# zcash/halo2

Hardware: AMD Instinct MI355X
Metric: Pallas MSM Mscalar-mults/s (+ Fp NTT Gbutterflies/s) at k=20 (higher is better)
Workload: dtype u256 (8x32-bit Montgomery limbs)

## Files before the change

halo2_amd/csrc/msm_fold.hip:

```cpp
#include "msm_internal.cuh"

namespace h2 {

template <int FB>
__global__ void __launch_bounds__(256) msm_finish_buckets(const u32 *__restrict__ heads, const u32 *__restrict__ starts,
                                                          u32 *__restrict__ buckets, u32 *__restrict__ heavy,
                                                          u32 total_buckets, u32 T, u32 div) {
    H2_LATENCY_STAGE();
    const u32 b = (blockIdx.x * blockDim.x + threadIdx.x) / kGroup;
    if (b >= total_buckets) return;
    const bool lead = (threadIdx.x & (kGroup - 1)) == 0;
    const u32 M = starts[total_buckets];
    T = eff_lanes(M, T, div);
    const u32 chunk = max(1u, (M + T - 1) / T);
    const u32 h0 = (starts[b] + chunk - 1) / chunk, h1 = (starts[b + 1] + chunk - 1) / chunk;
    if (h1 <= h0) return;
    if (h1 - h0 > kHeavy) {
        u32 slot = 0;
        if (lead) slot = atomicAdd(&heavy[1], 1u);
        slot = (u32)__builtin_amdgcn_mov_dpp((int)slot, 0, 0xf, 0xf, false);
        if (slot < kMaxHeavy) {
            if (lead) {
                heavy[2 + slot] = b;
                atomicAdd(&heavy[0], 1u);
// ... 99 lines not shown
        starts = H2_COLZ(starts, cs.starts);
        buckets9 = H2_COLZ(buckets9, cs.buckets);
        heavy = H2_COLZ(heavy, cs.heavy);
    }
    const u32 base = starts[0];
    const u32 M = starts[total_buckets] - base;
    T = eff_lanes(M, T, div);
    const u32 chunk = max(1u, (M + T - 1) / T);
    const u32 h0 = (starts[b] - base + chunk - 1) / chunk, h1 = (starts[b + 1] - base + chunk - 1) / chunk;
    if (h1 <= h0) return;
    if (h1 - h0 > kHeavy) {
        const u32 slot = atomicAdd(&heavy[1], 1u);
        if (slot < kMaxHeavy) {
            heavy[2 + slot] = b;
            atomicAdd(&heavy[0], 1u);
            return;
        }
    }
    xyzz9<FB> acc = xyzz9_load_raw<FB>(buckets9 + 36 * (size_t)b);
    for (u32 t = h0; t < h1; ++t) xyzz9_add<FB>(acc, xyzz9_load_raw<FB>(heads9 + 36 * (size_t)t));
    xyzz9_store_raw<FB>(buckets9 + 36 * (size_t)b, acc);
}
template <int FB>
__global__ void __launch_bounds__(256, 3) fold9_finish_heavy(const u32 *__restrict__ heads9, const u32 *__restrict__ starts, u32 *__restrict__ scratch9,
                                                          const u32 *__restrict__ heavy, u32 total_buckets, u32 T, u32 div, ColStride cs) {
    if (!cs.lowprio) H2_LATENCY_STAGE();
    __shared__ __attribute__((aligned(16))) u32 sh[32 * 36];
    if (gridDim.z > 1) {
        heavy = H2_COLZ(heavy, cs.heavy);
        heads9 = H2_COLZ(heads9, cs.heads);
        starts = H2_COLZ(starts, cs.starts);
        scratch9 = H2_COLZ(scratch9, cs.hscratch);
    }
    const u32 count = min(heavy[1], kMaxHeavy);
    const u32 base = starts[0];
    const u32 M = starts[total_buckets] - base;
    T = eff_lanes(M, T, div);
    const u32 chunk = max(1u, (M + T - 1) / T);
    for (u32 slot = blockIdx.y; slot < count; slot += gridDim.y) {
        const u32 b = heavy[2 + slot];
        const u32 h0 = (starts[b] - base + chunk - 1) / chunk, h1 = (starts[b + 1] - base + chunk - 1) / chunk;
        const u32 share = (h1 - h0 + kHeavyBlocks - 1) / kHeavyBlocks;
        const u32 lo = h0 + blockIdx.x * share, hi = min(h1, lo + share);
        xyzz9<FB> acc = fold9_quad_gather<FB, H2_FOLD_D>(heads9, hi > lo ? hi - lo : 0u, [lo](u32 k) { return lo + k; });
        acc = fold9_quads_sum<FB>(acc, sh);
        if (fold9_root() && (threadIdx.x & (kGroup - 1)) == 0) xyzz9_store_raw<FB>(scratch9 + 36 * ((size_t)slot * kHeavyBlocks + blockIdx.x), acc);
// ... 21 lines not shown
            if ((threadIdx.x & (kGroup - 1)) == 0) xyzz9_store_raw<FB>(buckets9 + 36 * (size_t)b, acc);
        }
        __syncthreads();
    }
}
template <int FB>
__global__ void __launch_bounds__(256, 3) fold9_rowcol(const u32 *__restrict__ buckets9, u32 *__restrict__ lines9, u32 S, u32 NR, ColStride cs) {
    if (!cs.lowprio) H2_LATENCY_STAGE();
    __shared__ __attribute__((aligned(16))) u32 sh[32 * 36];
    if (gridDim.z > 1) {
        buckets9 = H2_COLZ(buckets9, cs.buckets);
        lines9 = H2_COLZ(lines9, cs.lines);
    }
    const bool is_col = blockIdx.x < S;
    const u32 id = is_col ? blockIdx.x : blockIdx.x - S + 1;
    const u32 cnt = is_col ? NR : S;
    const u32 base = blockIdx.y * S * NR + (is_col ? id : id * S), step = is_col ? S : 1;
    xyzz9<FB> acc = fold9_quad_gather<FB, H2_FOLD_D>(buckets9, cnt, [base, step](u32 k) { return base + k * step; });
    acc = fold9_quads_sum<FB>(acc, sh);
    if (fold9_root() && (threadIdx.x & (kGroup - 1)) == 0)
        xyzz9_store_raw<FB>(lines9 + 36 * ((size_t)blockIdx.y * (S + NR) + (is_col ? id : S + id)), acc);
}
template <int FB>
__global__ void __launch_bounds__(256, 3) fold9_planes(const u32 *__restrict__ lines9, u32 *__restrict__ planes9, u32 *__restrict__ counter, u32 S, u32 NR,
                                                    int cb, u32 *__restrict__ out, int out_kind, int out_mont, ColOut co, ColStride cs) {
    if (!cs.lowprio) H2_LATENCY_STAGE();
    __shared__ __attribute__((aligned(16))) u32 sh[32 * 36];
    __shared__ u32 s_last;
    if (gridDim.z > 1) {
        lines9 = H2_COLZ(lines9, cs.lines);
        planes9 = H2_COLZ(planes9, cs.planes);
        counter = H2_COLZ(counter, cs.ctr);
        out = co.out[blockIdx.z];
    }
    const u32 t = blockIdx.x, planes = gridDim.x;
    const bool lead = (threadIdx.x & (kGroup - 1)) == 0;
    lines9 += 36 * (size_t)blockIdx.y * (S + NR);
    planes9 += 36 * (size_t)blockIdx.y * 32;
    counter += blockIdx.y;
    out += (out_kind == kOutSliceSum ? 32 : out_kind == H2_OUT_AFFINE ? 16 : 24) * (size_t)blockIdx.y;
    const u32 ncol = (int)t < cb ? S / 2 : (int)t == cb ? 1u : 0u, nrow = (int)t >= cb ? NR / 2 : 0u;
    const u32 jc = t, jr = t - (u32)cb;
    xyzz9<FB> acc = fold9_quad_gather<FB, H2_FOLD_D>(lines9, ncol + nrow, [=](u32 k) {
        if (k < ncol) {
            if ((int)jc == cb) return S - 1;
            return ((((k >> jc) << (jc + 1)) | (1u << jc) | (k & ((1u << jc) - 1u))) - 1u);
        }
        const u32 r = k - ncol;
        return S + (((r >> jr) << (jr + 1)) | (1u << jr) | (r & ((1u << jr) - 1u)));
    });
    acc = fold9_quads_sum<FB>(acc, sh);
    if (fold9_root()) {
        for (u32 k = 0; k < t; ++k) acc = xyzz9_dbl_wide<FB>(acc);
        if (lead) {
            xyzz9_store_raw<FB>(planes9 + 36 * (size_t)t, acc);
            __threadfence();
            s_last = atomicAdd(counter, 1u) == planes - 1 ? 1u : 0u;
        }
    }
    __syncthreads();
    if (!s_last) return;
    __threadfence();
    acc = fold9_quad_gather<FB, H2_FOLD_D>(planes9, planes, [](u32 k) { return k; });
    acc = fold9_quads_sum<FB>(acc, sh);
    if (!fold9_root()) return;
    const xyzz<FB> r = xyzz9_to_r256_wide<FB>(acc);
    if (!lead) return;
    *counter = 0;
    if (out_kind == kOutSliceSum) {
        xyzz_store<FB>(out, r);
        return;
    }
    if (out_kind == H2_OUT_AFFINE) {
        affine<FB> o = xyzz_to_affine<FB>(r);
        if (!out_mont) { o.x = fe_from_mont<FB>(o.x); o.y = fe_from_mont<FB>(o.y); }
        fe_store(out, o.x);
        fe_store(out + 8, o.y);
    } else {
        fe X, Y, Z;
        xyzz_to_jacobian<FB>(r, X, Y, Z);
        if (!out_mont) { X = fe_from_mont<FB>(X); Y = fe_from_mont<FB>(Y); Z = fe_from_mont<FB>(Z); }
        fe_store(out, X);
        fe_store(out + 8, Y);
        fe_store(out + 16, Z);
    }
}


template <int FB>
__global__ void __launch_bounds__(256) msm_reduce_segments(const u32 *__restrict__ buckets, u32 *__restrict__ partial,
// ... 57 lines not shown
    const size_t base = is_col ? id : (size_t)id * S, step = is_col ? S : 1;
    xyzz<FB> acc = xyzz_identity<FB>();
    for (u32 i = t; i < cnt; i += nl) {
        xyzz<FB> p = xyzz_load<FB>(buckets + 32 * (base + (size_t)i * step));
        xyzz_add_wide<FB>(acc, p);
    }
    if (lead) xyzz_store<FB>(sh + 32 * t, acc);
    __syncthreads();
    for (u32 off = nl / 2; off > 0; off >>= 1) {
        if (t < off) {
            xyzz<FB> a = xyzz_load<FB>(sh + 32 * t), b = xyzz_load<FB>(sh + 32 * (t + off));
            xyzz_add_wide<FB>(a, b);
            if (lead) xyzz_store<FB>(sh + 32 * t, a);
        }
        __syncthreads();
    }
    if (threadIdx.x == 0) {
        xyzz<FB> r = xyzz_load<FB>(sh);
        xyzz_store<FB>(wide + 32 * (is_col ? (size_t)id : (size_t)NR + id - 1), r);
    }
}

template <int FB>
__global__ void __launch_bounds__(64) msm_combine(const u32 *__restrict__ slice_sums, int slices, int c, u32 *__restrict__ out,
                                                  int out_kind, int out_mont, int extra_dbl, const u32 *__restrict__ addend, int addend_first) {
    H2_LATENCY_STAGE();
    if (threadIdx.x >= kGroup) return;
    if (gridDim.x > 1) {
        slice_sums += 32 * (size_t)blockIdx.x;
        out += (out_kind == H2_OUT_AFFINE ? 16 : 24) * (size_t)blockIdx.x;
        slices = 1;
    }
    xyzz9<FB> r9 = xyzz9_identity<FB>();
    for (int w = slices - 1; w >= 0; --w) {
        if (w != slices - 1)
            for (int k = 0; k < c; ++k) r9 = xyzz9_dbl_wide<FB>(r9);
        const xyzz9<FB> s9 = xyzz9_from_r256_wide<FB>(xyzz_load<FB>(slice_sums + 32 * (size_t)w));
        xyzz9_add_wide<FB>(r9, s9);
    }
    if (addend && addend_first) xyzz9_add_wide<FB>(r9, xyzz9_from_r256_wide<FB>(xyzz_load<FB>(addend)));
    for (int k = 0; k < extra_dbl; ++k) r9 = xyzz9_dbl_wide<FB>(r9);
    if (addend && !addend_first) xyzz9_add_wide<FB>(r9, xyzz9_from_r256_wide<FB>(xyzz_load<FB>(addend)));
    const xyzz<FB> r = xyzz9_to_r256_wide<FB>(r9);
    if (threadIdx.x != 0) return;
    if (out_kind == kOutSliceSum) {
        xyzz_store<FB>(out, r);
        return;
    }
    if (out_kind == H2_OUT_AFFINE) {
        affine<FB> a = xyzz_to_affine<FB>(r);
        if (!out_mont) { a.x = fe_from_mont<FB>(a.x); a.y = fe_from_mont<FB>(a.y); }
        fe_store(out, a.x);
        fe_store(out + 8, a.y);
    } else {
        fe X, Y, Z;
        xyzz_to_jacobian<FB>(r, X, Y, Z);
        if (!out_mont) { X = fe_from_mont<FB>(X); Y = fe_from_mont<FB>(Y); Z = fe_from_mont<FB>(Z); }
        fe_store(out, X);
        fe_store(out + 8, Y);
        fe_store(out + 16, Z);
    }
}

template <int FB>
__global__ void __launch_bounds__(64) msm_combine_ranges(RangeSums rs, int ranges, int slices, int c, u32 *__restrict__ out, int out_kind, int out_mont) {
    H2_LATENCY_STAGE();
    __shared__ __attribute__((aligned(16))) u32 sh[16 * 36];
    const int w = threadIdx.x / kGroup;
    const bool lead = (threadIdx.x & (kGroup - 1)) == 0;
    if (w < slices) {
        xyzz9<FB> acc = xyzz9_identity<FB>();
        for (int q = 0; q < ranges; ++q) xyzz9_add_wide<FB>(acc, xyzz9_from_r256_wide<FB>(xyzz_load<FB>(rs.p[q] + 32 * (size_t)w)));
        if (lead) xyzz9_store_raw<FB>(sh + 36 * w, acc);
    }
    __syncthreads();
    if (threadIdx.x >= kGroup) return;
    xyzz9<FB> r9 = xyzz9_identity<FB>();
    for (int s = slices - 1; s >= 0; --s) {
        if (s != slices - 1)
            for (int k = 0; k < c; ++k) r9 = xyzz9_dbl_wide<FB>(r9);
        xyzz9_add_wide<FB>(r9, xyzz9_load_raw<FB>(sh + 36 * s));
    }
    const xyzz<FB> r = xyzz9_to_r256_wide<FB>(r9);
    if (threadIdx.x != 0) return;
// ... 15 lines not shown

template __global__ void msm_finish_buckets<FP>(const u32 *__restrict__ heads, const u32 *__restrict__ starts,
                                                          u32 *__restrict__ buckets, u32 *__restrict__ heavy,
                                                          u32 total_buckets, u32 T, u32 div);
template __global__ void msm_finish_buckets<FQ>(const u32 *__restrict__ heads, const u32 *__restrict__ starts,
                                                          u32 *__restrict__ buckets, u32 *__restrict__ heavy,
                                                          u32 total_buckets, u32 T, u32 div);
template __global__ void msm_finish_heavy<FP>(const u32 *__restrict__ heads, const u32 *__restrict__ starts,
                                                        u32 *__restrict__ scratch, const u32 *__restrict__ heavy,
                                                        u32 total_buckets, u32 T, u32 div);
template __global__ void msm_finish_heavy<FQ>(const u32 *__restrict__ heads, const u32 *__restrict__ starts,
                                                        u32 *__restrict__ scratch, const u32 *__restrict__ heavy,
                                                        u32 total_buckets, u32 T, u32 div);
template __global__ void msm_finish_heavy2<FP>(const u32 *__restrict__ scratch, u32 *__restrict__ buckets,
                                                        const u32 *__restrict__ heavy);
template __global__ void msm_finish_heavy2<FQ>(const u32 *__restrict__ scratch, u32 *__restrict__ buckets,
                                                        const u32 *__restrict__ heavy);
template __global__ void msm_bucket_add<FP>(u32 *__restrict__ total, const u32 *__restrict__ part, u32 nb);
template __global__ void msm_bucket_add<FQ>(u32 *__restrict__ total, const u32 *__restrict__ part, u32 nb);
template __global__ void fold9_finish<FP>(const u32 *__restrict__ heads9, const u32 *__restrict__ starts, u32 *__restrict__ buckets9,
                                                    u32 *__restrict__ heavy, u32 total_buckets, u32 T, u32 div, ColStride cs);
template __global__ void fold9_finish<FQ>(const u32 *__restrict__ heads9, const u32 *__restrict__ starts, u32 *__restrict__ buckets9,
                                                    u32 *__restrict__ heavy, u32 total_buckets, u32 T, u32 div, ColStride cs);
template __global__ void fold9_finish_heavy<FP>(const u32 *__restrict__ heads9, const u32 *__restrict__ starts, u32 *__restrict__ scratch9,
                                                          const u32 *__restrict__ heavy, u32 total_buckets, u32 T, u32 div, ColStride cs);
template __global__ void fold9_finish_heavy<FQ>(const u32 *__restrict__ heads9, const u32 *__restrict__ starts, u32 *__restrict__ scratch9,
                                                          const u32 *__restrict__ heavy, u32 total_buckets, u32 T, u32 div, ColStride cs);
template __global__ void fold9_finish_heavy2<FP>(const u32 *__restrict__ scratch9, u32 *__restrict__ buckets9, const u32 *__restrict__ heavy,
                                                             ColStride cs);
template __global__ void fold9_finish_heavy2<FQ>(const u32 *__restrict__ scratch9, u32 *__restrict__ buckets9, const u32 *__restrict__ heavy,
                                                             ColStride cs);
template __global__ void fold9_rowcol<FP>(const u32 *__restrict__ buckets9, u32 *__restrict__ lines9, u32 S, u32 NR, ColStride cs);
template __global__ void fold9_rowcol<FQ>(const u32 *__restrict__ buckets9, u32 *__restrict__ lines9, u32 S, u32 NR, ColStride cs);
template __global__ void fold9_planes<FP>(const u32 *__restrict__ lines9, u32 *__restrict__ planes9, u32 *__restrict__ counter, u32 S, u32 NR,
                                                    int cb, u32 *__restrict__ out, int out_kind, int out_mont, ColOut co, ColStride cs);
template __global__ void fold9_planes<FQ>(const u32 *__restrict__ lines9, u32 *__restrict__ planes9, u32 *__restrict__ counter, u32 S, u32 NR,
                                                    int cb, u32 *__restrict__ out, int out_kind, int out_mont, ColOut co, ColStride cs);
template __global__ void msm_reduce_segments<FP>(const u32 *__restrict__ buckets, u32 *__restrict__ partial,
                                                           u32 NB, u32 total_segments, int seg);
template __global__ void msm_reduce_segments<FQ>(const u32 *__restrict__ buckets, u32 *__restrict__ partial,
                                                           u32 NB, u32 total_segments, int seg);
template __global__ void msm_sum_slice<FP>(const u32 *__restrict__ partial, u32 *__restrict__ out, u32 per_slice,
                                                     u32 share);
template __global__ void msm_sum_slice<FQ>(const u32 *__restrict__ partial, u32 *__restrict__ out, u32 per_slice,
                                                     u32 share);
template __global__ void msm_rowcol_sums<FP>(const u32 *__restrict__ buckets, u32 *__restrict__ wide, u32 S, u32 NR);
template __global__ void msm_rowcol_sums<FQ>(const u32 *__restrict__ buckets, u32 *__restrict__ wide, u32 S, u32 NR);
template __global__ void msm_combine<FP>(const u32 *__restrict__ slice_sums, int slices, int c, u32 *__restrict__ out,
                                                  int out_kind, int out_mont, int extra_dbl, const u32 *__restrict__ addend, int addend_first);
template __global__ void msm_combine<FQ>(const u32 *__restrict__ slice_sums, int slices, int c, u32 *__restrict__ out,
                                                  int out_kind, int out_mont, int extra_dbl, const u32 *__restrict__ addend, int addend_first);
template __global__ void msm_combine_ranges<FP>(RangeSums rs, int ranges, int slices, int c, u32 *__restrict__ out, int out_kind, int out_mont);
template __global__ void msm_combine_ranges<FQ>(RangeSums rs, int ranges, int slices, int c, u32 *__restrict__ out, int out_kind, int out_mont);

}
```

halo2_amd/csrc/msm_generic.hip:

```cpp
#include <cassert>

#include "msm_internal.cuh"

namespace h2 {

namespace {

struct Group {
    u32 w0 = 0, ns = 0;
    u32 tb = 0;
    GroupSort gs;
    Sort2 p2;
    size_t cap = 0;
    size_t emax = 0;
    size_t plan_words = 0;
    u32 B1 = 0;
    u32 T = 0;
    size_t ent_off = 0;
    size_t starts_off = 0;
    size_t bucket_off = 0;
};

bool group_geometry(u32 cols, u32 nb, Group &g) {
    int lb = 0;
// ... 34 lines not shown
        g.cap = cap;
        g.B1 = (cols + S - 1) / S;
        g.plan_words = ((size_t)nh * 2 + 1 + 64 + (((size_t)kMaxBig * (kBigChunks + 1)) << lowb) + 3) & ~(size_t)3;
        return true;
    }
    return false;
}

}

template <int FB, int FS>
int msm_generic_grouped(MsmContext &cx, const MsmArgs &a, const MsmShape &sh, size_t scalars_n, u32 lanes, hipStream_t st) {
    static const bool on = [] { const char *e = ab_env("H2_GENERIC_GROUPED"); return !(e && atoi(e) == 0); }();
    static const size_t min_n = [] { const char *e = ab_env("H2_GENERIC_GROUPED_MIN"); return e ? (size_t)atol(e) : ((size_t)1 << 18) + 1; }();
    if (!on || scalars_n < min_n || sh.c < 8 || sh.c > kMaxC || sh.W < 3 || sh.W > 16 || sh.NB < 128) return H2_ERR_BATCH_SHAPE;
    const u32 m = (u32)scalars_n, cols = 2 * m, W = (u32)sh.W, NB = sh.NB, c = (u32)sh.c;
    int rc;
    static const bool fold_late = [] { const char *e = ab_env("H2_GG_FOLD_LATE"); return e && atoi(e) == 1; }();
    static const int lowprio = [] { const char *e = ab_env("H2_GG_LOWPRIO"); return e ? atoi(e) : 0; }();
    static const int acc_block = [] { const char *e = ab_env("H2_GG_ACC_BLOCK"); return e && atoi(e) == 256 ? 256 : 512; }();
    static const int skip = [] { const char *e = ab_env("H2_GG_SKIP"); return e ? atoi(e) : 0; }();
    static const bool big_all = [] { const char *e = ab_env("H2_GG_BIG"); return !(e && atoi(e) == 0); }();
    static const int form_env = [] { const char *e = ab_env("H2_GG_FORM"); return e ? atoi(e) : 0; }();
    const bool throughput = form_env == 2 || (form_env != 1 && scalars_n < ((size_t)1 << 22) && msm_other_generic_in_flight(&cx));
    int sizes[MsmContext::kMaxGroups] = {0, 0, 0, 0}, G = 0;
    static const std::vector<int> env_sizes = [] {
        std::vector<int> v;
        if (const char *e = ab_env("H2_GENERIC_GROUPS"))
            for (const char *p = e; *p;) {
                v.push_back(atoi(p));
                while (*p && *p != ',') ++p;
                if (*p == ',') ++p;
            }
        return v;
    }();
    {
        int sum = 0;
        for (int v : env_sizes) sum += v;
        if (!env_sizes.empty() && env_sizes.size() <= (size_t)MsmContext::kMaxGroups && sum == (int)W && *std::min_element(env_sizes.begin(), env_sizes.end()) >= 1) {
            for (int v : env_sizes) sizes[G++] = v;
        } else {
            if (throughput) {
                sizes[0] = (int)W;
                G = 1;
            } else {
                const int last = std::max(1, (int)W * 2 / 9), mid = last, top = (int)W - last - mid;
// ... 104 lines not shown
        H2_HIP(hipStreamWaitEvent(st, cx.gev[2 + 3 * G], 0));
    }
    H2_HIP(hipEventRecord(ev_fork, st));
    H2_HIP(hipStreamWaitEvent(fold_s(0), ev_fork, 0));
    hipLaunchKernelGGL((msm_bases_to_m9_glv<FB>), dim3((m + 255) / 256), dim3(256), 0, fold_s(0), (const u32 *)a.d_bases, cx.bases9.as<u32>(), m);
    H2_HIP(hipEventRecord(ev_conv, fold_s(0)));
    hipLaunchKernelGGL((msm_glv_digits<FS>), dim3((m + 255) / 256), dim3(256), 0, st, (const u32 *)a.d_scalars, digits, m, row, (int)c, (int)W, mont ? 1 : 0);

    size_t heads_off = 0;
    u32 *heads_of[MsmContext::kMaxGroups];
    for (int g = 0; g < G; ++g) {
        heads_of[g] = heads_all + 36 * heads_off;
        heads_off += grp[g].T;
    }
    auto sort_group = [&](int g, hipStream_t s_) {
        const Group &q = grp[g];
        u32 *bin_count = cx.plan.as<u32>(), *bin_start = bin_count + q.gs.nh, *big = bin_start + q.gs.nh + 1, *gcnt = big + 64;
        u32 *starts = cx.starts.as<u32>() + q.starts_off, *entries = cx.entries.as<u32>() + q.ent_off, *heavy = cx.heavy.as<u32>() + (size_t)g * (kMaxHeavy + 2);
        const size_t nbk = (size_t)1 << q.gs.lowb;
        hipLaunchKernelGGL(msm_d1_count, dim3(q.B1), dim3(512), q.gs.nh * 4, s_, (const uint16_t *)digits, q.gs, hist1);
        hipLaunchKernelGGL(msm_s1_prefix, dim3((q.gs.nh + 15) / 16), dim3(1024), 0, s_, hist1, bin_count, q.B1, q.gs.nh, heavy, big, starts + q.tb + 1, cs);
        hipLaunchKernelGGL(msm_d1_scatter, dim3(q.B1), dim3(512), ((size_t)q.gs.nh * 3 + 1 + (size_t)q.gs.S * q.ns) * 4, s_, (const uint16_t *)digits, q.gs,
                           (const u32 *)hist1, (const u32 *)bin_count, bin_start, tagged);
        hipLaunchKernelGGL(msm_s2_bins, dim3(q.gs.nh), dim3(1024), (nbk * 2 + q.cap) * 4, s_, (const u32 *)tagged, (const uint16_t *)nullptr, (const u32 *)bin_start, q.p2,
                           q.tb, (u32)q.cap, starts, entries, big, (big_all || !g) ? kMaxBig : 0u, buckets_all + 36 * q.bucket_off, cs);
        if (!big_all && g) return;
        hipLaunchKernelGGL(msm_s2_big_count, dim3(kBigChunks, kMaxBig), dim3(256), nbk * 4, s_, (const u32 *)tagged, (const uint16_t *)nullptr, (const u32 *)bin_start, q.p2,
                           (const u32 *)big, gcnt, cs);
        hipLaunchKernelGGL(msm_s2_big_prefix, dim3(kMaxBig), dim3(256), nbk * 4, s_, (const u32 *)bin_start, q.p2, q.tb, (const u32 *)big, gcnt, starts, cs);
        hipLaunchKernelGGL(msm_s2_big_scatter, dim3(kBigChunks, kMaxBig), dim3(256), nbk * 4, s_, (const u32 *)tagged, (const uint16_t *)nullptr, (const u32 *)bin_start, q.p2,
                           (const u32 *)big, (const u32 *)gcnt, entries, cs);
    };
    auto fold_group = [&](int g, hipStream_t s_) {
        const Group &q = grp[g];
        const u32 *starts = cx.starts.as<u32>() + q.starts_off;
        u32 *gbuckets = buckets_all + 36 * q.bucket_off, *heavy = cx.heavy.as<u32>() + (size_t)g * (kMaxHeavy + 2);
        u32 *hscr = cx.hscratch.as<u32>() + (size_t)g * kMaxHeavy * kHeavyBlocks * 36;
        const int sk = g < G - 1 ? skip : 0, lp = g < G - 1 ? lowprio : 0;
        ColStride cs = cs0, csf = cs0, csh = cs0, csr = cs0, csp = cs0;
        csf.lowprio = (lp & 1) ? 1u : 0u;
        csh.lowprio = (lp & 2) ? 1u : 0u;
        csr.lowprio = (lp & 4) ? 1u : 0u;
        csp.lowprio = (lp & 8) ? 1u : 0u;
        (void)cs;
        if (!(sk & 1)) hipLaunchKernelGGL((fold9_finish<FB>), dim3((q.tb + 255) / 256), dim3(256), 0, s_, (const u32 *)heads_of[g], starts, gbuckets, heavy, q.tb, q.T, lane_div, csf);
        if (!(sk & 2)) hipLaunchKernelGGL((fold9_finish_heavy<FB>), dim3(kHeavyBlocks, kHeavyRows), dim3(256), 0, s_, (const u32 *)heads_of[g], starts, hscr, (const u32 *)heavy, q.tb, q.T, lane_div, csh);
        if (!(sk & 2)) hipLaunchKernelGGL((fold9_finish_heavy2<FB>), dim3(kHeavyRows), dim3(64), 0, s_, (const u32 *)hscr, gbuckets, (const u32 *)heavy, csh);
        if (!(sk & 4)) hipLaunchKernelGGL((fold9_rowcol<FB>), dim3(wideS + wideNR - 1, q.ns), dim3(256), 0, s_, (const u32 *)gbuckets, lines9 + 36 * (size_t)q.w0 * (wideS + wideNR), wideS, wideNR, csr);
        if (!(sk & 8)) hipLaunchKernelGGL((fold9_planes<FB>), dim3(c - 1, q.ns), dim3(256), 0, s_, (const u32 *)(lines9 + 36 * (size_t)q.w0 * (wideS + wideNR)), planes9 + 36 * (size_t)q.w0 * 32,
                           cx.fold_ctr.as<u32>() + q.w0, wideS, wideNR, cb, ssums + 32 * (size_t)q.w0, kOutSliceSum, mont, co, csp);
    };

    sort_group(0, st);
    if (G > 1) {
        H2_HIP(hipEventRecord(ev_sorted(0), st));
        H2_HIP(hipStreamWaitEvent(sort_s, ev_sorted(0), 0));
    }
    for (int g = 1; g < G; ++g) {
        sort_group(g, sort_s);
        H2_HIP(hipEventRecord(ev_sorted(g), sort_s));
    }
    H2_HIP(hipStreamWaitEvent(st, ev_conv, 0));
    for (int g = 0; g < G; ++g) {
        const Group &q = grp[g];
        if (g) H2_HIP(hipStreamWaitEvent(st, ev_sorted(g), 0));
        if (acc_block == 512)
            hipLaunchKernelGGL((msm_accumulate<FB, false, true, 512>), dim3(q.T / 512), dim3(512), lds_fence ? 65536 : 0, st, pts, (const u32 *)nullptr, 0xFFFFFFFFu,
                               (const u32 *)(cx.entries.as<u32>() + q.ent_off), (const u32 *)(cx.starts.as<u32>() + q.starts_off), heads_of[g],
                               buckets_all + 36 * q.bucket_off, q.tb, q.T, lane_div, cs);
        else
        hipLaunchKernelGGL((msm_accumulate<FB, false, true>), dim3(q.T / 256), dim3(256), 0, st, pts, (const u32 *)nullptr, 0xFFFFFFFFu,
                           (const u32 *)(cx.entries.as<u32>() + q.ent_off), (const u32 *)(cx.starts.as<u32>() + q.starts_off), heads_of[g],
                           buckets_all + 36 * q.bucket_off, q.tb, q.T, lane_div, cs);
        if (g < G - 1 && !fold_late) {
            hipStream_t fs = fold_s(g);
            H2_HIP(hipEventRecord(ev_acc(g), st));
            H2_HIP(hipStreamWaitEvent(fs, ev_acc(g), 0));
            fold_group(g, fs);
            if (g) H2_HIP(hipStreamWaitEvent(fs, ev_chain(g - 1), 0));
            if (!(skip & 16)) hipLaunchKernelGGL((msm_combine<FB>), dim3(1), dim3(64), lds_fence ? 100 * 1024 : 0, fs, (const u32 *)(ssums + 32 * (size_t)q.w0), (int)q.ns, (int)c, ssums + 32 * (size_t)(W + g), kOutSliceSum, 1,
                               (int)(c * grp[g + 1].ns), g ? (const u32 *)(ssums + 32 * (size_t)(W + g - 1)) : (const u32 *)nullptr, 1);
            H2_HIP(hipEventRecord(ev_chain(g), fs));
        }
    }
    if (fold_late)
        for (int g = 0; g < G - 1; ++g) {
            fold_group(g, st);
            hipLaunchKernelGGL((msm_combine<FB>), dim3(1), dim3(64), 0, st, (const u32 *)(ssums + 32 * (size_t)grp[g].w0), (int)grp[g].ns, (int)c, ssums + 32 * (size_t)(W + g), kOutSliceSum, 1,
                               (int)(c * grp[g + 1].ns), g ? (const u32 *)(ssums + 32 * (size_t)(W + g - 1)) : (const u32 *)nullptr, 1);
        }
    fold_group(G - 1, st);
    if (G > 1 && !fold_late) H2_HIP(hipStreamWaitEvent(st, ev_chain(G - 2), 0));
    hipLaunchKernelGGL((msm_combine<FB>), dim3(1), dim3(64), 0, st, (const u32 *)(ssums + 32 * (size_t)grp[G - 1].w0), (int)grp[G - 1].ns, (int)c, (u32 *)a.d_out, a.out_kind,
                       mont ? 1 : 0, 0, G > 1 ? (const u32 *)(ssums + 32 * (size_t)(W + G - 2)) : (const u32 *)nullptr, 1);
    H2_HIP(hipGetLastError());
    if (st != caller) {
        H2_HIP(hipEventRecord(cx.gev[3 + 3 * G], st));
        H2_HIP(hipStreamWaitEvent(caller, cx.gev[3 + 3 * G], 0));
        st = caller;
    }
    if (!cx.gdone) H2_HIP(hipEventCreateWithFlags(&cx.gdone, hipEventDisableTiming));
    H2_HIP(hipEventRecord(cx.gdone, st));
    cx.gpending = true;
    return H2_OK;
}

template int msm_generic_grouped<FP, FQ>(MsmContext &cx, const MsmArgs &a, const MsmShape &sh, size_t scalars_n, u32 lanes, hipStream_t st);
template int msm_generic_grouped<FQ, FP>(MsmContext &cx, const MsmArgs &a, const MsmShape &sh, size_t scalars_n, u32 lanes, hipStream_t st);

}
```

halo2_amd/csrc/msm_internal.cuh:

```cuda
#pragma once
#include <algorithm>
#include <atomic>
#include <cmath>
#include <cstdlib>
#include <cstring>
#include <map>
#include <memory>
#include <mutex>
#include <thread>
#include <vector>

#include "common.h"
#include "curve_wide.cuh"
#include "curve9.cuh"
#include "curve9_wide.cuh"
#include "glv.cuh"
#include "host_field.h"
namespace h2 {

extern std::atomic<double> g_lane_fraction;
extern std::atomic<size_t> g_pipe_chunk;
static constexpr int kMaxC = 16;
static constexpr int kMaxCShared = 20;
static constexpr u32 kZeroCode = 0xFFFFu;
// ... 449 lines not shown
                                                        u32 total_buckets, u32 T, u32 div);
extern template __global__ void msm_finish_heavy<FQ>(const u32 *__restrict__ heads, const u32 *__restrict__ starts,
                                                        u32 *__restrict__ scratch, const u32 *__restrict__ heavy,
                                                        u32 total_buckets, u32 T, u32 div);
template <int FB>
__global__ void __launch_bounds__(64) msm_finish_heavy2(const u32 *__restrict__ scratch, u32 *__restrict__ buckets,
                                                        const u32 *__restrict__ heavy);
extern template __global__ void msm_finish_heavy2<FP>(const u32 *__restrict__ scratch, u32 *__restrict__ buckets,
                                                        const u32 *__restrict__ heavy);
extern template __global__ void msm_finish_heavy2<FQ>(const u32 *__restrict__ scratch, u32 *__restrict__ buckets,
                                                        const u32 *__restrict__ heavy);
template <int FB>
__global__ void __launch_bounds__(256) msm_bucket_add(u32 *__restrict__ total, const u32 *__restrict__ part, u32 nb);
extern template __global__ void msm_bucket_add<FP>(u32 *__restrict__ total, const u32 *__restrict__ part, u32 nb);
extern template __global__ void msm_bucket_add<FQ>(u32 *__restrict__ total, const u32 *__restrict__ part, u32 nb);
template <int FB>
__global__ void __launch_bounds__(256) fold9_finish(const u32 *__restrict__ heads9, const u32 *__restrict__ starts, u32 *__restrict__ buckets9,
                                                    u32 *__restrict__ heavy, u32 total_buckets, u32 T, u32 div, ColStride cs);
extern template __global__ void fold9_finish<FP>(const u32 *__restrict__ heads9, const u32 *__restrict__ starts, u32 *__restrict__ buckets9,
                                                    u32 *__restrict__ heavy, u32 total_buckets, u32 T, u32 div, ColStride cs);
extern template __global__ void fold9_finish<FQ>(const u32 *__restrict__ heads9, const u32 *__restrict__ starts, u32 *__restrict__ buckets9,
                                                    u32 *__restrict__ heavy, u32 total_buckets, u32 T, u32 div, ColStride cs);
template <int FB>
__global__ void __launch_bounds__(256, 3) fold9_finish_heavy(const u32 *__restrict__ heads9, const u32 *__restrict__ starts, u32 *__restrict__ scratch9,
                                                          const u32 *__restrict__ heavy, u32 total_buckets, u32 T, u32 div, ColStride cs);
extern template __global__ void fold9_finish_heavy<FP>(const u32 *__restrict__ heads9, const u32 *__restrict__ starts, u32 *__restrict__ scratch9,
                                                          const u32 *__restrict__ heavy, u32 total_buckets, u32 T, u32 div, ColStride cs);
extern template __global__ void fold9_finish_heavy<FQ>(const u32 *__restrict__ heads9, const u32 *__restrict__ starts, u32 *__restrict__ scratch9,
                                                          const u32 *__restrict__ heavy, u32 total_buckets, u32 T, u32 div, ColStride cs);
template <int FB>
__global__ void __launch_bounds__(64, 3) fold9_finish_heavy2(const u32 *__restrict__ scratch9, u32 *__restrict__ buckets9, const u32 *__restrict__ heavy,
                                                             ColStride cs);
extern template __global__ void fold9_finish_heavy2<FP>(const u32 *__restrict__ scratch9, u32 *__restrict__ buckets9, const u32 *__restrict__ heavy,
                                                             ColStride cs);
extern template __global__ void fold9_finish_heavy2<FQ>(const u32 *__restrict__ scratch9, u32 *__restrict__ buckets9, const u32 *__restrict__ heavy,
                                                             ColStride cs);
template <int FB>
__global__ void __launch_bounds__(256, 3) fold9_rowcol(const u32 *__restrict__ buckets9, u32 *__restrict__ lines9, u32 S, u32 NR, ColStride cs);
extern template __global__ void fold9_rowcol<FP>(const u32 *__restrict__ buckets9, u32 *__restrict__ lines9, u32 S, u32 NR, ColStride cs);
extern template __global__ void fold9_rowcol<FQ>(const u32 *__restrict__ buckets9, u32 *__restrict__ lines9, u32 S, u32 NR, ColStride cs);
template <int FB>
__global__ void __launch_bounds__(256, 3) fold9_planes(const u32 *__restrict__ lines9, u32 *__restrict__ planes9, u32 *__restrict__ counter, u32 S, u32 NR,
                                                    int cb, u32 *__restrict__ out, int out_kind, int out_mont, ColOut co, ColStride cs);
extern template __global__ void fold9_planes<FP>(const u32 *__restrict__ lines9, u32 *__restrict__ planes9, u32 *__restrict__ counter, u32 S, u32 NR,
                                                    int cb, u32 *__restrict__ out, int out_kind, int out_mont, ColOut co, ColStride cs);
extern template __global__ void fold9_planes<FQ>(const u32 *__restrict__ lines9, u32 *__restrict__ planes9, u32 *__restrict__ counter, u32 S, u32 NR,
                                                    int cb, u32 *__restrict__ out, int out_kind, int out_mont, ColOut co, ColStride cs);
template <int FB>
__global__ void __launch_bounds__(256) msm_reduce_segments(const u32 *__restrict__ buckets, u32 *__restrict__ partial,
                                                           u32 NB, u32 total_segments, int seg);
extern template __global__ void msm_reduce_segments<FP>(const u32 *__restrict__ buckets, u32 *__restrict__ partial,
                                                           u32 NB, u32 total_segments, int seg);
extern template __global__ void msm_reduce_segments<FQ>(const u32 *__restrict__ buckets, u32 *__restrict__ partial,
                                                           u32 NB, u32 total_segments, int seg);
template <int FB>
__global__ void __launch_bounds__(256) msm_sum_slice(const u32 *__restrict__ partial, u32 *__restrict__ out, u32 per_slice,
                                                     u32 share);
extern template __global__ void msm_sum_slice<FP>(const u32 *__restrict__ partial, u32 *__restrict__ out, u32 per_slice,
                                                     u32 share);
extern template __global__ void msm_sum_slice<FQ>(const u32 *__restrict__ partial, u32 *__restrict__ out, u32 per_slice,
                                                     u32 share);
template <int FB>
__global__ void __launch_bounds__(256) msm_rowcol_sums(const u32 *__restrict__ buckets, u32 *__restrict__ wide, u32 S, u32 NR);
extern template __global__ void msm_rowcol_sums<FP>(const u32 *__restrict__ buckets, u32 *__restrict__ wide, u32 S, u32 NR);
// ... 15 lines not shown
```

Baseline: 1152.

## Add alternative fold kernels and reorder sort/accumulate scheduling in generic MSM

Adds several new MSM fold variants, each behind an env switch. One finishes buckets per head lane using a binary search. A quad-group finish variant prefetches the next head. A multi-line rowcol kernel uses 16 lanes per line with a shared-memory tree reduction. A fused planes+Horner tail kernel drops the separate combine launch. Group 0 accumulation is also scheduled before the sorts of later groups so it can overlap them. Most paths are on by default (fused tail is off), which changes launch shapes and stream ordering and brings new synchronization risk.

Measured after the change: 1152, median of 2. About the same (-0.1%).

```diff
diff --git a/halo2_amd/csrc/msm_fold.hip b/halo2_amd/csrc/msm_fold.hip
--- a/halo2_amd/csrc/msm_fold.hip
+++ b/halo2_amd/csrc/msm_fold.hip
@@ -145,6 +145,71 @@
     xyzz9_store_raw<FB>(buckets9 + 36 * (size_t)b, acc);
 }
 template <int FB>
+__global__ void __launch_bounds__(256) fold9_finish_heads(const u32 *__restrict__ heads9, const u32 *__restrict__ starts, u32 *__restrict__ buckets9,
+                                                          u32 *__restrict__ heavy, u32 total_buckets, u32 T, u32 div, ColStride cs) {
+    if (!cs.lowprio) H2_LATENCY_STAGE();
+    const u32 t = blockIdx.x * blockDim.x + threadIdx.x;
+    const u32 base = starts[0];
+    const u32 M = starts[total_buckets] - base;
+    T = eff_lanes(M, T, div);
+    const u32 chunk = max(1u, (M + T - 1) / T);
+    if (t >= T || (u64)t * chunk >= M) return;
+    const u32 p = t * chunk;
+    u32 lo = 0, hi = total_buckets;
+    while (hi - lo > 1) {
+        const u32 mid = (lo + hi) >> 1;
+        if (starts[mid] - base <= p) lo = mid; else hi = mid;
+    }
+    const u32 b = lo;
+    const u32 h0 = (starts[b] - base + chunk - 1) / chunk, h1 = (starts[b + 1] - base + chunk - 1) / chunk;
+    if (t != h0) return;
+    if (h1 - h0 > kHeavy) {
+        const u32 slot = atomicAdd(&heavy[1], 1u);
+        if (slot < kMaxHeavy) {
+            heavy[2 + slot] = b;
+            atomicAdd(&heavy[0], 1u);
+            return;
+        }
+    }
+    xyzz9<FB> acc = xyzz9_load_raw<FB>(buckets9 + 36 * (size_t)b);
+    for (u32 k = h0; k < h1; ++k) xyzz9_add<FB>(acc, xyzz9_load_raw<FB>(heads9 + 36 * (size_t)k));
+    xyzz9_store_raw<FB>(buckets9 + 36 * (size_t)b, acc);
+}
+template <int FB>
+__global__ void __launch_bounds__(256) fold9_finish_quad(const u32 *__restrict__ heads9, const u32 *__restrict__ starts, u32 *__restrict__ buckets9,
+                                                         u32 *__restrict__ heavy, u32 total_buckets, u32 T, u32 div) {
+    H2_LATENCY_STAGE();
+    const u32 b = (blockIdx.x * blockDim.x + threadIdx.x) / kGroup;
+    if (b >= total_buckets) return;
+    const bool lead = (threadIdx.x & (kGroup - 1)) == 0;
+    const u32 base = starts[0];
+    const u32 M = starts[total_buckets] - base;
+    T = eff_lanes(M, T, div);
+    const u32 chunk = max(1u, (M + T - 1) / T);
+    const u32 h0 = (starts[b] - base + chunk - 1) / chunk, h1 = (starts[b + 1] - base + chunk - 1) / chunk;
+    if (h1 <= h0) return;
+    if (h1 - h0 > kHeavy) {
+        u32 slot = 0;
+        if (lead) slot = atomicAdd(&heavy[1], 1u);
+        slot = (u32)__builtin_amdgcn_mov_dpp((int)slot, 0, 0xf, 0xf, false);
+        if (slot < kMaxHeavy) {
+            if (lead) {
+                heavy[2 + slot] = b;
+                atomicAdd(&heavy[0], 1u);
+            }
+            return;
+        }
+    }
+    xyzz9<FB> acc = xyzz9_load_raw<FB>(buckets9 + 36 * (size_t)b);
+    xyzz9<FB> nxt = xyzz9_load_raw<FB>(heads9 + 36 * (size_t)h0);
+    for (u32 t = h0; t < h1; ++t) {
+        const xyzz9<FB> p = nxt;
+        if (t + 1 < h1) nxt = xyzz9_load_raw<FB>(heads9 + 36 * (size_t)(t + 1));
+        xyzz9_add_wide<FB>(acc, p);
+    }
+    if (lead) xyzz9_store_raw<FB>(buckets9 + 36 * (size_t)b, acc);
+}
+template <int FB>
 __global__ void __launch_bounds__(256, 3) fold9_finish_heavy(const u32 *__restrict__ heads9, const u32 *__restrict__ starts, u32 *__restrict__ scratch9,
                                                           const u32 *__restrict__ heavy, u32 total_buckets, u32 T, u32 div, ColStride cs) {
     if (!cs.lowprio) H2_LATENCY_STAGE();
@@ -212,8 +277,36 @@
         xyzz9_store_raw<FB>(lines9 + 36 * ((size_t)blockIdx.y * (S + NR) + (is_col ? id : S + id)), acc);
 }
 template <int FB>
-__global__ void __launch_bounds__(256, 3) fold9_planes(const u32 *__restrict__ lines9, u32 *__restrict__ planes9, u32 *__restrict__ counter, u32 S, u32 NR,
-                                                    int cb, u32 *__restrict__ out, int out_kind, int out_mont, ColOut co, ColStride cs) {
+__global__ void __launch_bounds__(256, 3) fold9_rowcol_lanes(const u32 *__restrict__ buckets9, u32 *__restrict__ lines9, u32 S, u32 NR, ColStride cs) {
+    if (!cs.lowprio) H2_LATENCY_STAGE();
+    constexpr u32 kLineLanes = 16;
+    __shared__ __attribute__((aligned(16))) u32 sh[256 * 36];
+    const u32 sub = threadIdx.x & (kLineLanes - 1), line = blockIdx.x * (256 / kLineLanes) + threadIdx.x / kLineLanes;
+    const bool live = line < S + NR - 1;
+    const bool is_col = line < S;
+    const u32 id = is_col ? line : line - S + 1;
+    const u32 cnt = live ? (is_col ? NR : S) : 0u;
+    const u32 base = blockIdx.y * S * NR + (is_col ? id : id * S), step = is_col ? S : 1;
+    xyzz9<FB> acc = xyzz9_identity<FB>();
+    if (sub < cnt) {
+        xyzz9<FB> nxt = xyzz9_load_raw<FB>(buckets9 + 36 * (size_t)(base + sub * step));
+        for (u32 k = sub; k < cnt; k += kLineLanes) {
+            const xyzz9<FB> p = nxt;
+            if (k + kLineLanes < cnt) nxt = xyzz9_load_raw<FB>(buckets9 + 36 * (size_t)(base + (k + kLineLanes) * step));
+            xyzz9_add<FB>(acc, p);
+        }
+    }
+    for (u32 off = kLineLanes / 2; off > 0; off >>= 1) {
+        if (sub >= off && sub < 2 * off) xyzz9_store_raw<FB>(sh + 36 * (size_t)threadIdx.x, acc);
+        __syncthreads();
+        if (sub < off) xyzz9_add<FB>(acc, xyzz9_load_raw<FB>(sh + 36 * (size_t)(threadIdx.x + off)));
+        __syncthreads();
+    }
+    if (live && sub == 0) xyzz9_store_raw<FB>(lines9 + 36 * ((size_t)blockIdx.y * (S + NR) + (is_col ? id : S + id)), acc);
+}
+template <int FB>
+__device__ __forceinline__ bool fold9_planes_slice(const u32 *__restrict__ lines9, u32 *__restrict__ planes9, u32 *__restrict__ &counter, u32 S, u32 NR,
+                                                   int cb, u32 *__restrict__ &out, int out_kind, const ColOut &co, const ColStride &cs, xyzz<FB> &r) {
     if (!cs.lowprio) H2_LATENCY_STAGE();
     __shared__ __attribute__((aligned(16))) u32 sh[32 * 36];
     __shared__ u32 s_last;
@@ -249,13 +342,20 @@
         }
     }
     __syncthreads();
-    if (!s_last) return;
+    if (!s_last) return false;
     __threadfence();
     acc = fold9_quad_gather<FB, H2_FOLD_D>(planes9, planes, [](u32 k) { return k; });
     acc = fold9_quads_sum<FB>(acc, sh);
-    if (!fold9_root()) return;
-    const xyzz<FB> r = xyzz9_to_r256_wide<FB>(acc);
-    if (!lead) return;
+    if (!fold9_root()) return false;
+    r = xyzz9_to_r256_wide<FB>(acc);
+    return true;
+}
+template <int FB>
+__global__ void __launch_bounds__(256, 3) fold9_planes(const u32 *__restrict__ lines9, u32 *__restrict__ planes9, u32 *__restrict__ counter, u32 S, u32 NR,
+                                                    int cb, u32 *__restrict__ out, int out_kind, int out_mont, ColOut co, ColStride cs) {
+    xyzz<FB> r;
+    if (!fold9_planes_slice<FB>(lines9, planes9, counter, S, NR, cb, out, out_kind, co, cs, r)) return;
+    if ((threadIdx.x & (kGroup - 1)) != 0) return;
     *counter = 0;
     if (out_kind == kOutSliceSum) {
         xyzz_store<FB>(out, r);
@@ -359,6 +459,9 @@
 }
 
 template <int FB>
+__device__ __forceinline__ void horner_emit(const u32 *__restrict__ slice_sums, int slices, int c, u32 *__restrict__ out,
+                                            int out_kind, int out_mont, int extra_dbl, const u32 *__restrict__ addend, int addend_first);
+template <int FB>
 __global__ void __launch_bounds__(64) msm_combine(const u32 *__restrict__ slice_sums, int slices, int c, u32 *__restrict__ out,
                                                   int out_kind, int out_mont, int extra_dbl, const u32 *__restrict__ addend, int addend_first) {
     H2_LATENCY_STAGE();
@@ -368,6 +471,11 @@
         out += (out_kind == H2_OUT_AFFINE ? 16 : 24) * (size_t)blockIdx.x;
         slices = 1;
     }
+    horner_emit<FB>(slice_sums, slices, c, out, out_kind, out_mont, extra_dbl, addend, addend_first);
+}
+template <int FB>
+__device__ __forceinline__ void horner_emit(const u32 *__restrict__ slice_sums, int slices, int c, u32 *__restrict__ out,
+                                            int out_kind, int out_mont, int extra_dbl, const u32 *__restrict__ addend, int addend_first) {
     xyzz9<FB> r9 = xyzz9_identity<FB>();
     for (int w = slices - 1; w >= 0; --w) {
         if (w != slices - 1)
@@ -397,6 +505,29 @@
         fe_store(out + 8, Y);
         fe_store(out + 16, Z);
     }
+}
+
+template <int FB>
+__global__ void __launch_bounds__(256, 3) fold9_planes_horner(const u32 *__restrict__ lines9, u32 *__restrict__ planes9, u32 *__restrict__ counter, u32 S, u32 NR,
+                                                              int cb, u32 *__restrict__ slice_sums, u32 *__restrict__ group_counter, int c, u32 *__restrict__ result,
+                                                              int out_kind, int out_mont, const u32 *__restrict__ addend) {
+    xyzz<FB> r;
+    ColOut co = {};
+    ColStride cs = {};
+    u32 *out = slice_sums;
+    if (!fold9_planes_slice<FB>(lines9, planes9, counter, S, NR, cb, out, kOutSliceSum, co, cs, r)) return;
+    u32 last = 0;
+    if ((threadIdx.x & (kGroup - 1)) == 0) {
+        *counter = 0;
+        xyzz_store<FB>(out, r);
+        __threadfence();
+        last = atomicAdd(group_counter, 1u) == gridDim.y - 1 ? 1u : 0u;
+    }
+    last = (u32)__builtin_amdgcn_mov_dpp((int)last, 0, 0xf, 0xf, false);
+    if (!last) return;
+    __threadfence();
+    if (threadIdx.x == 0) *group_counter = 0;
+    horner_emit<FB>(slice_sums, (int)gridDim.y, c, result, out_kind, out_mont, 0, addend, 1);
 }
 
 template <int FB>
@@ -458,6 +589,20 @@
                                                     u32 *__restrict__ heavy, u32 total_buckets, u32 T, u32 div, ColStride cs);
 template __global__ void fold9_finish<FQ>(const u32 *__restrict__ heads9, const u32 *__restrict__ starts, u32 *__restrict__ buckets9,
                                                     u32 *__restrict__ heavy, u32 total_buckets, u32 T, u32 div, ColStride cs);
+template __global__ void fold9_finish_heads<FP>(const u32 *__restrict__ heads9, const u32 *__restrict__ starts, u32 *__restrict__ buckets9,
+                                                          u32 *__restrict__ heavy, u32 total_buckets, u32 T, u32 div, ColStride cs);
+template __global__ void fold9_finish_heads<FQ>(const u32 *__restrict__ heads9, const u32 *__restrict__ starts, u32 *__restrict__ buckets9,
+                                                          u32 *__restrict__ heavy, u32 total_buckets, u32 T, u32 div, ColStride cs);
+template __global__ void fold9_finish_quad<FP>(const u32 *__restrict__ heads9, const u32 *__restrict__ starts, u32 *__restrict__ buckets9,
+                                                         u32 *__restrict__ heavy, u32 total_buckets, u32 T, u32 div);
+template __global__ void fold9_finish_quad<FQ>(const u32 *__restrict__ heads9, const u32 *__restrict__ starts, u32 *__restrict__ buckets9,
+                                                         u32 *__restrict__ heavy, u32 total_buckets, u32 T, u32 div);
+template __global__ void fold9_planes_horner<FP>(const u32 *__restrict__ lines9, u32 *__restrict__ planes9, u32 *__restrict__ counter, u32 S, u32 NR,
+                                                              int cb, u32 *__restrict__ slice_sums, u32 *__restrict__ group_counter, int c, u32 *__restrict__ result,
+                                                              int out_kind, int out_mont, const u32 *__restrict__ addend);
+template __global__ void fold9_planes_horner<FQ>(const u32 *__restrict__ lines9, u32 *__restrict__ planes9, u32 *__restrict__ counter, u32 S, u32 NR,
+                                                              int cb, u32 *__restrict__ slice_sums, u32 *__restrict__ group_counter, int c, u32 *__restrict__ result,
+                                                              int out_kind, int out_mont, const u32 *__restrict__ addend);
 template __global__ void fold9_finish_heavy<FP>(const u32 *__restrict__ heads9, const u32 *__restrict__ starts, u32 *__restrict__ scratch9,
                                                           const u32 *__restrict__ heavy, u32 total_buckets, u32 T, u32 div, ColStride cs);
 template __global__ void fold9_finish_heavy<FQ>(const u32 *__restrict__ heads9, const u32 *__restrict__ starts, u32 *__restrict__ scratch9,
@@ -468,6 +613,8 @@
                                                              ColStride cs);
 template __global__ void fold9_rowcol<FP>(const u32 *__restrict__ buckets9, u32 *__restrict__ lines9, u32 S, u32 NR, ColStride cs);
 template __global__ void fold9_rowcol<FQ>(const u32 *__restrict__ buckets9, u32 *__restrict__ lines9, u32 S, u32 NR, ColStride cs);
+template __global__ void fold9_rowcol_lanes<FP>(const u32 *__restrict__ buckets9, u32 *__restrict__ lines9, u32 S, u32 NR, ColStride cs);
+template __global__ void fold9_rowcol_lanes<FQ>(const u32 *__restrict__ buckets9, u32 *__restrict__ lines9, u32 S, u32 NR, ColStride cs);
 template __global__ void fold9_planes<FP>(const u32 *__restrict__ lines9, u32 *__restrict__ planes9, u32 *__restrict__ counter, u32 S, u32 NR,
                                                     int cb, u32 *__restrict__ out, int out_kind, int out_mont, ColOut co, ColStride cs);
 template __global__ void fold9_planes<FQ>(const u32 *__restrict__ lines9, u32 *__restrict__ planes9, u32 *__restrict__ counter, u32 S, u32 NR,
diff --git a/halo2_amd/csrc/msm_generic.hip b/halo2_amd/csrc/msm_generic.hip
--- a/halo2_amd/csrc/msm_generic.hip
+++ b/halo2_amd/csrc/msm_generic.hip
@@ -80,6 +80,11 @@
     static const int skip = [] { const char *e = ab_env("H2_GG_SKIP"); return e ? atoi(e) : 0; }();
     static const bool big_all = [] { const char *e = ab_env("H2_GG_BIG"); return !(e && atoi(e) == 0); }();
     static const int form_env = [] { const char *e = ab_env("H2_GG_FORM"); return e ? atoi(e) : 0; }();
+    static const bool acc_first = [] { const char *e = ab_env("H2_GG_ACC_FIRST"); return !(e && atoi(e) == 0); }();
+    static const bool fused_tail = [] { const char *e = ab_env("H2_GG_FUSED_TAIL"); return e && atoi(e) == 1; }();
+    static const bool rowcol_lanes = [] { const char *e = ab_env("H2_GG_ROWCOL_LANES"); return !(e && atoi(e) == 0); }();
+    static const bool finish_heads = [] { const char *e = ab_env("H2_GG_FINISH_HEADS"); return !(e && atoi(e) == 0); }();
+    static const bool finish_quad = [] { const char *e = ab_env("H2_GG_FINISH_QUAD"); return !(e && atoi(e) == 0); }();
     const bool throughput = form_env == 2 || (form_env != 1 && scalars_n < ((size_t)1 << 22) && msm_other_generic_in_flight(&cx));
     int sizes[MsmContext::kMaxGroups] = {0, 0, 0, 0}, G = 0;
     static const std::vector<int> env_sizes = [] {
@@ -230,6 +235,7 @@
         hipLaunchKernelGGL(msm_s1_prefix, dim3((q.gs.nh + 15) / 16), dim3(1024), 0, s_, hist1, bin_count, q.B1, q.gs.nh, heavy, big, starts + q.tb + 1, cs);
         hipLaunchKernelGGL(msm_d1_scatter, dim3(q.B1), dim3(512), ((size_t)q.gs.nh * 3 + 1 + (size_t)q.gs.S * q.ns) * 4, s_, (const uint16_t *)digits, q.gs,
                            (const u32 *)hist1, (const u32 *)bin_count, bin_start, tagged);
+        if (!g && acc_first) (void)hipStreamWaitEvent(s_, ev_conv, 0);
         hipLaunchKernelGGL(msm_s2_bins, dim3(q.gs.nh), dim3(1024), (nbk * 2 + q.cap) * 4, s_, (const u32 *)tagged, (const uint16_t *)nullptr, (const u32 *)bin_start, q.p2,
                            q.tb, (u32)q.cap, starts, entries, big, (big_all || !g) ? kMaxBig : 0u, buckets_all + 36 * q.bucket_off, cs);
         if (!big_all && g) return;
@@ -251,27 +257,31 @@
         csr.lowprio = (lp & 4) ? 1u : 0u;
         csp.lowprio = (lp & 8) ? 1u : 0u;
         (void)cs;
+        if (g == G - 1 && !throughput && finish_quad)
+            hipLaunchKernelGGL((fold9_finish_quad<FB>), dim3((q.tb * kGroup + 255) / 256), dim3(256), 0, s_, (const u32 *)heads_of[g], starts, gbuckets, heavy, q.tb, q.T, lane_div);
+        else if (finish_heads && !(sk & 1))
+            hipLaunchKernelGGL((fold9_finish_heads<FB>), dim3((q.T + 255) / 256), dim3(256), 0, s_, (const u32 *)heads_of[g], starts, gbuckets, heavy, q.tb, q.T, lane_div, csf);
+        else
         if (!(sk & 1)) hipLaunchKernelGGL((fold9_finish<FB>), dim3((q.tb + 255) / 256), dim3(256), 0, s_, (const u32 *)heads_of[g], starts, gbuckets, heavy, q.tb, q.T, lane_div, csf);
         if (!(sk & 2)) hipLaunchKernelGGL((fold9_finish_heavy<FB>), dim3(kHeavyBlocks, kHeavyRows), dim3(256), 0, s_, (const u32 *)heads_of[g], starts, hscr, (const u32 *)heavy, q.tb, q.T, lane_div, csh);
         if (!(sk & 2)) hipLaunchKernelGGL((fold9_finish_heavy2<FB>), dim3(kHeavyRows), dim3(64), 0, s_, (const u32 *)hscr, gbuckets, (const u32 *)heavy, csh);
+        if (!(sk & 4) && rowcol_lanes && (g < G - 1 || throughput))
+            hipLaunchKernelGGL((fold9_rowcol_lanes<FB>), dim3((wideS + wideNR - 1 + 15) / 16, q.ns), dim3(256), 0, s_, (const u32 *)gbuckets, lines9 + 36 * (size_t)q.w0 * (wideS + wideNR), wideS, wideNR, csr);
+        else
         if (!(sk & 4)) hipLaunchKernelGGL((fold9_rowcol<FB>), dim3(wideS + wideNR - 1, q.ns), dim3(256), 0, s_, (const u32 *)gbuckets, lines9 + 36 * (size_t)q.w0 * (wideS + wideNR), wideS, wideNR, csr);
+        if (g == G - 1 && fused_tail) {
+            if (G > 1 && !fold_late) (void)hipStreamWaitEvent(s_, ev_chain(G - 2), 0);
+            hipLaunchKernelGGL((fold9_planes_horner<FB>), dim3(c - 1, q.ns), dim3(256), 0, s_, (const u32 *)(lines9 + 36 * (size_t)q.w0 * (wideS + wideNR)), planes9 + 36 * (size_t)q.w0 * 32,
+                               cx.fold_ctr.as<u32>() + q.w0, wideS, wideNR, cb, ssums + 32 * (size_t)q.w0, cx.fold_ctr.as<u32>() + kMaxCols * 8, (int)c, (u32 *)a.d_out, a.out_kind, mont ? 1 : 0,
+                               G > 1 ? (const u32 *)(ssums + 32 * (size_t)(W + G - 2)) : (const u32 *)nullptr);
+            return;
+        }
         if (!(sk & 8)) hipLaunchKernelGGL((fold9_planes<FB>), dim3(c - 1, q.ns), dim3(256), 0, s_, (const u32 *)(lines9 + 36 * (size_t)q.w0 * (wideS + wideNR)), planes9 + 36 * (size_t)q.w0 * 32,
                            cx.fold_ctr.as<u32>() + q.w0, wideS, wideNR, cb, ssums + 32 * (size_t)q.w0, kOutSliceSum, mont, co, csp);
     };
 
-    sort_group(0, st);
-    if (G > 1) {
-        H2_HIP(hipEventRecord(ev_sorted(0), st));
-        H2_HIP(hipStreamWaitEvent(sort_s, ev_sorted(0), 0));
-    }
-    for (int g = 1; g < G; ++g) {
-        sort_group(g, sort_s);
-        H2_HIP(hipEventRecord(ev_sorted(g), sort_s));
-    }
-    H2_HIP(hipStreamWaitEvent(st, ev_conv, 0));
-    for (int g = 0; g < G; ++g) {
+    auto accumulate_group = [&](int g) {
         const Group &q = grp[g];
-        if (g) H2_HIP(hipStreamWaitEvent(st, ev_sorted(g), 0));
         if (acc_block == 512)
             hipLaunchKernelGGL((msm_accumulate<FB, false, true, 512>), dim3(q.T / 512), dim3(512), lds_fence ? 65536 : 0, st, pts, (const u32 *)nullptr, 0xFFFFFFFFu,
                                (const u32 *)(cx.entries.as<u32>() + q.ent_off), (const u32 *)(cx.starts.as<u32>() + q.starts_off), heads_of[g],
@@ -280,6 +290,28 @@
         hipLaunchKernelGGL((msm_accumulate<FB, false, true>), dim3(q.T / 256), dim3(256), 0, st, pts, (const u32 *)nullptr, 0xFFFFFFFFu,
                            (const u32 *)(cx.entries.as<u32>() + q.ent_off), (const u32 *)(cx.starts.as<u32>() + q.starts_off), heads_of[g],
                            buckets_all + 36 * q.bucket_off, q.tb, q.T, lane_div, cs);
+    };
+    sort_group(0, st);
+    if (G > 1) H2_HIP(hipEventRecord(ev_sorted(0), st));
+    if (!acc_first) {
+        if (G > 1) H2_HIP(hipStreamWaitEvent(sort_s, ev_sorted(0), 0));
+        for (int g = 1; g < G; ++g) {
+            sort_group(g, sort_s);
+            H2_HIP(hipEventRecord(ev_sorted(g), sort_s));
+        }
+        H2_HIP(hipStreamWaitEvent(st, ev_conv, 0));
+    }
+    for (int g = 0; g < G; ++g) {
+        const Group &q = grp[g];
+        if (g) H2_HIP(hipStreamWaitEvent(st, ev_sorted(g), 0));
+        accumulate_group(g);
+        if (!g && acc_first && G > 1) {
+            H2_HIP(hipStreamWaitEvent(sort_s, ev_sorted(0), 0));
+            for (int h = 1; h < G; ++h) {
+                sort_group(h, sort_s);
+                H2_HIP(hipEventRecord(ev_sorted(h), sort_s));
+            }
+        }
         if (g < G - 1 && !fold_late) {
             hipStream_t fs = fold_s(g);
             H2_HIP(hipEventRecord(ev_acc(g), st));
@@ -298,9 +330,11 @@
                                (int)(c * grp[g + 1].ns), g ? (const u32 *)(ssums + 32 * (size_t)(W + g - 1)) : (const u32 *)nullptr, 1);
         }
     fold_group(G - 1, st);
+    if (!fused_tail) {
     if (G > 1 && !fold_late) H2_HIP(hipStreamWaitEvent(st, ev_chain(G - 2), 0));
     hipLaunchKernelGGL((msm_combine<FB>), dim3(1), dim3(64), 0, st, (const u32 *)(ssums + 32 * (size_t)grp[G - 1].w0), (int)grp[G - 1].ns, (int)c, (u32 *)a.d_out, a.out_kind,
                        mont ? 1 : 0, 0, G > 1 ? (const u32 *)(ssums + 32 * (size_t)(W + G - 2)) : (const u32 *)nullptr, 1);
+    }
     H2_HIP(hipGetLastError());
     if (st != caller) {
         H2_HIP(hipEventRecord(cx.gev[3 + 3 * G], st));
diff --git a/halo2_amd/csrc/msm_internal.cuh b/halo2_amd/csrc/msm_internal.cuh
--- a/halo2_amd/csrc/msm_internal.cuh
+++ b/halo2_amd/csrc/msm_internal.cuh
@@ -495,6 +495,30 @@
 extern template __global__ void fold9_finish<FQ>(const u32 *__restrict__ heads9, const u32 *__restrict__ starts, u32 *__restrict__ buckets9,
                                                     u32 *__restrict__ heavy, u32 total_buckets, u32 T, u32 div, ColStride cs);
 template <int FB>
+__global__ void __launch_bounds__(256) fold9_finish_heads(const u32 *__restrict__ heads9, const u32 *__restrict__ starts, u32 *__restrict__ buckets9,
+                                                          u32 *__restrict__ heavy, u32 total_buckets, u32 T, u32 div, ColStride cs);
+extern template __global__ void fold9_finish_heads<FP>(const u32 *__restrict__ heads9, const u32 *__restrict__ starts, u32 *__restrict__ buckets9,
+                                                          u32 *__restrict__ heavy, u32 total_buckets, u32 T, u32 div, ColStride cs);
+extern template __global__ void fold9_finish_heads<FQ>(const u32 *__restrict__ heads9, const u32 *__restrict__ starts, u32 *__restrict__ buckets9,
+                                                          u32 *__restrict__ heavy, u32 total_buckets, u32 T, u32 div, ColStride cs);
+template <int FB>
+__global__ void __launch_bounds__(256) fold9_finish_quad(const u32 *__restrict__ heads9, const u32 *__restrict__ starts, u32 *__restrict__ buckets9,
+                                                         u32 *__restrict__ heavy, u32 total_buckets, u32 T, u32 div);
+extern template __global__ void fold9_finish_quad<FP>(const u32 *__restrict__ heads9, const u32 *__restrict__ starts, u32 *__restrict__ buckets9,
+                                                         u32 *__restrict__ heavy, u32 total_buckets, u32 T, u32 div);
+extern template __global__ void fold9_finish_quad<FQ>(const u32 *__restrict__ heads9, const u32 *__restrict__ starts, u32 *__restrict__ buckets9,
+                                                         u32 *__restrict__ heavy, u32 total_buckets, u32 T, u32 div);
+template <int FB>
+__global__ void __launch_bounds__(256, 3) fold9_planes_horner(const u32 *__restrict__ lines9, u32 *__restrict__ planes9, u32 *__restrict__ counter, u32 S, u32 NR,
+                                                              int cb, u32 *__restrict__ slice_sums, u32 *__restrict__ group_counter, int c, u32 *__restrict__ result,
+                                                              int out_kind, int out_mont, const u32 *__restrict__ addend);
+extern template __global__ void fold9_planes_horner<FP>(const u32 *__restrict__ lines9, u32 *__restrict__ planes9, u32 *__restrict__ counter, u32 S, u32 NR,
+                                                              int cb, u32 *__restrict__ slice_sums, u32 *__restrict__ group_counter, int c, u32 *__restrict__ result,
+                                                              int out_kind, int out_mont, const u32 *__restrict__ addend);
+extern template __global__ void fold9_planes_horner<FQ>(const u32 *__restrict__ lines9, u32 *__restrict__ planes9, u32 *__restrict__ counter, u32 S, u32 NR,
+                                                              int cb, u32 *__restrict__ slice_sums, u32 *__restrict__ group_counter, int c, u32 *__restrict__ result,
+                                                              int out_kind, int out_mont, const u32 *__restrict__ addend);
+template <int FB>
 __global__ void __launch_bounds__(256, 3) fold9_finish_heavy(const u32 *__restrict__ heads9, const u32 *__restrict__ starts, u32 *__restrict__ scratch9,
                                                           const u32 *__restrict__ heavy, u32 total_buckets, u32 T, u32 div, ColStride cs);
 extern template __global__ void fold9_finish_heavy<FP>(const u32 *__restrict__ heads9, const u32 *__restrict__ starts, u32 *__restrict__ scratch9,
@@ -513,6 +537,10 @@
 extern template __global__ void fold9_rowcol<FP>(const u32 *__restrict__ buckets9, u32 *__restrict__ lines9, u32 S, u32 NR, ColStride cs);
 extern template __global__ void fold9_rowcol<FQ>(const u32 *__restrict__ buckets9, u32 *__restrict__ lines9, u32 S, u32 NR, ColStride cs);
 template <int FB>
+__global__ void __launch_bounds__(256, 3) fold9_rowcol_lanes(const u32 *__restrict__ buckets9, u32 *__restrict__ lines9, u32 S, u32 NR, ColStride cs);
+extern template __global__ void fold9_rowcol_lanes<FP>(const u32 *__restrict__ buckets9, u32 *__restrict__ lines9, u32 S, u32 NR, ColStride cs);
+extern template __global__ void fold9_rowcol_lanes<FQ>(const u32 *__restrict__ buckets9, u32 *__restrict__ lines9, u32 S, u32 NR, ColStride cs);
+template <int FB>
 __global__ void __launch_bounds__(256, 3) fold9_planes(const u32 *__restrict__ lines9, u32 *__restrict__ planes9, u32 *__restrict__ counter, u32 S, u32 NR,
                                                     int cb, u32 *__restrict__ out, int out_kind, int out_mont, ColOut co, ColStride cs);
 extern template __global__ void fold9_planes<FP>(const u32 *__restrict__ lines9, u32 *__restrict__ planes9, u32 *__restrict__ counter, u32 S, u32 NR,
```
